# lukedan/libfluid

Hardware: AMD Instinct MI355X
Metric: particle_steps_per_sec (higher is better)
Workload: dtype f32

## Files before the change

### include/libfluid_amd.h

```cpp
#ifndef LIBFLUID_AMD_H
#define LIBFLUID_AMD_H

#include <stddef.h>
#include <stdint.h>

#ifdef __cplusplus
extern "C" {
#endif

typedef struct lfa_sim lfa_sim;

enum {
	LFA_OK = 0,
	LFA_E_INVALID = -1,
	LFA_E_NO_DEVICE = -2,
	LFA_E_HIP = -3,
	LFA_E_OOM = -4,
	LFA_E_NAN = -5,
	LFA_E_UNSUPPORTED = -6,
	LFA_W_PCG_NOT_CONVERGED = 1
};

enum { LFA_PIC = 0, LFA_FLIP_BLEND = 1, LFA_APIC = 2 };
enum { LFA_P2G_LDS_BINNED = 0, LFA_P2G_GLOBAL_ATOMIC = 1 };
// ... 80 lines not shown
int lfa_p2g(lfa_sim *s);
int lfa_add_gravity(lfa_sim *s, double dt);
int lfa_build_system(lfa_sim *s, double dt);
int lfa_download_abits(lfa_sim *s, uint8_t *bits, uint64_t n);
int lfa_download_rhs(lfa_sim *s, double *b, uint64_t n);
int lfa_download_precon(lfa_sim *s, double *precon, uint64_t n);
int lfa_apply_preconditioner(lfa_sim *s, const double *r, double *z, uint64_t n);
int lfa_apply_a(lfa_sim *s, const double *v, double *out, uint64_t n);
int lfa_pcg_solve(lfa_sim *s, double dt, double *residual, uint64_t *iterations);
int lfa_download_pressure(lfa_sim *s, double *p, uint64_t n);
int lfa_upload_pressure(lfa_sim *s, const double *p, uint64_t n);
int lfa_apply_pressure(lfa_sim *s, double dt);
int lfa_extrapolate(lfa_sim *s);
int lfa_g2p(lfa_sim *s);
int lfa_cfl(lfa_sim *s, double *out);

int lfa_step_hot(lfa_sim *s, double dt, double *residual, uint64_t *iterations);

int lfa_clear_sources(lfa_sim *s);
int lfa_add_source(lfa_sim *s, const int32_t *xyz, uint64_t k, const double velocity[3], uint64_t target_density_cubic_root,
                   int active, int coerce_velocity);
int lfa_update_sources(lfa_sim *s, uint64_t *n_seeded);
int lfa_update_sources_rng(lfa_sim *s, uint64_t *rng_state, int flags, uint64_t *n_seeded, double *positions,
                           uint64_t positions_capacity);
int lfa_set_source_rng(lfa_sim *s, int on, uint64_t rng_state, int flags);
int lfa_get_source_rng(const lfa_sim *s, int *on, uint64_t *rng_state);
int lfa_source_last(const lfa_sim *s, uint64_t out[3]);
int lfa_advect_collide(lfa_sim *s, double dt);
int lfa_correct_collide(lfa_sim *s, double dt);
int lfa_advect(lfa_sim *s, double dt);
int lfa_correct(lfa_sim *s, double dt);
int lfa_collide(lfa_sim *s);
int lfa_time_step(lfa_sim *s, double dt, double *residual, uint64_t *iterations);
#define LFA_NUM_STEP_TIMERS 16
int lfa_get_step_timings(lfa_sim *s, double ms[LFA_NUM_STEP_TIMERS]);
int lfa_set_step_overlap(lfa_sim *s, int on);
int lfa_correct_collide_begin(lfa_sim *s, double dt);
int lfa_correct_collide_end(lfa_sim *s);
int lfa_correct_collide_undo(lfa_sim *s);

int lfa_dist_unique_id(void *id128);
int lfa_dist_init_rccl(lfa_sim *s, int rank, int nranks, const void *id128, const int32_t *layer_bounds);
typedef struct lfa_hub lfa_hub;
lfa_hub *lfa_dist_local_hub_create(int nranks);
void lfa_dist_local_hub_destroy(lfa_hub *h);
int lfa_dist_init_local(lfa_sim *s, lfa_hub *h, int rank, const int32_t *layer_bounds);
int lfa_dist_init_shm(lfa_sim *s, const char *name, int rank, int nranks, const int32_t *layer_bounds);
int lfa_dist_get_slab(const lfa_sim *s, int32_t *lo, int32_t *hi);
int lfa_dist_abandon(lfa_sim *s);

typedef struct lfa_voxels lfa_voxels;
enum { LFA_VOX_INTERIOR = 0, LFA_VOX_EXTERIOR = 1, LFA_VOX_SURFACE = 2 };
int lfa_voxels_create(lfa_voxels **out, const uint64_t size[3], const double grid_offset[3], double cell_size, int device);
void lfa_voxels_destroy(lfa_voxels *v);
const char *lfa_voxels_last_error(const lfa_voxels *v);
int lfa_voxels_info(const lfa_voxels *v, int32_t grid_min[3], uint64_t size[3], double grid_offset[3], double *cell_size);
int lfa_voxels_upload(lfa_voxels *v, const uint8_t *types);
int lfa_voxels_download(lfa_voxels *v, uint8_t *types);
int lfa_voxels_voxelize_triangles(lfa_voxels *v, const double *positions, uint64_t n_vertices, const void *indices,
                                  int index_bytes, uint64_t n_indices);
int lfa_voxels_mark_exterior(lfa_voxels *v);
int lfa_voxelize_mesh(lfa_voxels **out, const double *positions, uint64_t n_vertices, const void *indices, int index_bytes,
                      uint64_t n_indices, double cell_size, const double ref_grid_offset[3], int device);
int lfa_voxels_count(lfa_voxels *v, int include_interior, int include_surface, const int64_t *ref_grid_size, uint64_t *count);
int lfa_voxels_cells(lfa_voxels *v, int include_interior, int include_surface, const int64_t *ref_grid_size, int32_t *xyz,
                     uint64_t capacity, uint64_t *count);
// ... 70 lines not shown
```

### libfluid_amd/__init__.py

```python
import ctypes as C
import os

import numpy as np

from . import scenes
from .scenes import CELL_DTYPE, PARTICLE_DTYPE

HERE = os.path.dirname(os.path.abspath(__file__))
LIB_PATH = os.path.join(HERE, "libfluid_amd.so")

PIC, FLIP_BLEND, APIC = 0, 1, 2
P2G_LDS_BINNED, P2G_GLOBAL_ATOMIC = 0, 1
PRECOND_MIC0_TILED, PRECOND_MIC0_EXACT, PRECOND_MULTILEVEL, PRECOND_MULTIGRID = 0, 1, 2, 3
PCG_F32, PCG_F64 = 0, 1
SEED_DRAW_LTR, SEED_COLLECTIVE = 1, 2
OK, W_PCG_NOT_CONVERGED = 0, 1
NUM_TIMERS = 10
NUM_STEP_TIMERS = 16
STEP_TIMER_NAMES = ["advect_collide", "bin", "p2g", "p2g_scatter_kernel", "build_system", "pcg_loop", "apply_pressure",
                    "correct_cell_index", "correct_tiled_kernel", "correct_collide", "extrapolate", "g2p", "time_step",
                    "pcg_iterations", "pcg_iteration_mean", "overlapped"]
TIMER_NAMES = ["bin", "p2g", "gravity", "build_system", "pcg_loop", "apply_pressure", "extrapolate", "g2p",
               "p2g_scatter_kernel", "pcg_iteration_mean"]

# ... 124 lines not shown
    "lfa_set_solid_from_voxels": (_int, [_vp, _vp, _int, _int]),
    "lfa_mesher_create": (_int, [C.POINTER(_vp), _vp, _vp, _dbl, _dbl, _u64, _int]),
    "lfa_mesher_create_window": (_int, [C.POINTER(_vp), _vp, _vp, _dbl, _dbl, _u64, _u64, _u64, _int]),
    "lfa_mesher_window": (_int, [_vp, C.POINTER(_u64), C.POINTER(_u64), C.POINTER(_u64), C.POINTER(_u64)]),
    "lfa_mesher_sample_ids": (_int, [_vp, _vp, _vp, _u64, _dbl]),
    "lfa_mesher_rebase": (_int, [_vp, _u64]),
    "lfa_mesher_destroy": (None, [_vp]),
    "lfa_mesher_last_error": (C.c_char_p, [_vp]),
    "lfa_mesher_sample": (_int, [_vp, _vp, _u64, _dbl]),
    "lfa_mesher_sample_sim": (_int, [_vp, _vp, _dbl]),
    "lfa_mesher_download_values": (_int, [_vp, _vp]),
    "lfa_mesher_upload_values": (_int, [_vp, _vp]),
    "lfa_mesher_marching_cubes": (_int, [_vp, C.POINTER(_u64), C.POINTER(_u64)]),
    "lfa_mesher_download_mesh": (_int, [_vp, _vp, _vp]),
    "lfa_mesher_normals": (_int, [_vp]),
    "lfa_mesher_download_normals": (_int, [_vp, _vp]),
    "lfa_mesher_normals_time": (_int, [_vp, C.POINTER(_dbl)]),
    "lfa_mesher_boundary_size": (_int, [_vp, C.POINTER(_u64), C.POINTER(_u64)]),
    "lfa_mesher_download_boundary": (_int, [_vp, _vp, _vp]),
    "lfa_mesher_window_normals": (_int, [_vp, _vp, _vp, _u64]),
    "lfa_mesher_window_normals_from": (_int, [_vp, _vp]),
    "lfa_mesher_vertex_velocities": (_int, [_vp, _vp, C.POINTER(_u64)]),
    "lfa_mesher_vertex_velocities_collective": (_int, [_vp, _vp, C.POINTER(_u64 * 2)]),
    "lfa_mesher_download_velocities": (_int, [_vp, _vp]),
    "lfa_mesher_velocities_time": (_int, [_vp, C.POINTER(_dbl)]),
    "lfa_clear_sources": (_int, [_vp]),
    "lfa_add_source": (_int, [_vp, _vp, _u64, _vp, _u64, _int, _int]),
    "lfa_update_sources": (_int, [_vp, C.POINTER(_u64)]),
    "lfa_update_sources_rng": (_int, [_vp, C.POINTER(_u64), _int, C.POINTER(_u64), _vp, _u64]),
    "lfa_set_source_rng": (_int, [_vp, _int, _u64, _int]),
    "lfa_get_source_rng": (_int, [_vp, C.POINTER(_int), C.POINTER(_u64)]),
    "lfa_source_last": (_int, [_vp, C.POINTER(_u64 * 3)]),
    "lfa_advect_collide": (_int, [_vp, _dbl]),
    "lfa_advect": (_int, [_vp, _dbl]),
    "lfa_correct": (_int, [_vp, _dbl]),
    "lfa_collide": (_int, [_vp]),
    "lfa_correct_collide": (_int, [_vp, _dbl]),
    "lfa_time_step": (_int, [_vp, _dbl, C.POINTER(_dbl), C.POINTER(_u64)]),
    "lfa_get_step_timings": (_int, [_vp, C.POINTER(_dbl * NUM_STEP_TIMERS)]),
    "lfa_set_step_overlap": (_int, [_vp, _int]),
    "lfa_get_correction_stats": (_int, [_vp, C.POINTER(_u64 * 2)]),
    "lfa_get_correction_stats_ex": (_int, [_vp, C.POINTER(_u64 * 3)]),
    "lfa_correct_collide_begin": (_int, [_vp, _dbl]),
    "lfa_correct_collide_end": (_int, [_vp]),
    "lfa_correct_collide_undo": (_int, [_vp]),
    "lfa_dist_unique_id": (_int, [_vp]),
    "lfa_dist_init_rccl": (_int, [_vp, _int, _int, _vp, _vp]),
    "lfa_dist_local_hub_create": (_vp, [_int]),
    "lfa_dist_local_hub_destroy": (None, [_vp]),
    "lfa_dist_init_local": (_int, [_vp, _vp, _int, _vp]),
    "lfa_dist_init_shm": (_int, [_vp, C.c_char_p, _int, _int, _vp]),
    "lfa_dist_get_slab": (_int, [_vp, C.POINTER(C.c_int32), C.POINTER(C.c_int32)]),
    "lfa_dist_abandon": (_int, [_vp]),
}
KERNELS = {"spmv_dot": 0, "axpy_max": 1, "mic_apply_dot": 2, "update_s": 3, "p2g_scatter": 4, "p2g_finalize": 5,
           "g2p": 6, "bin": 7, "mic_fine": 8, "coarse_levels": 9, "pcg_a": 10, "pcg_b": 11,
           "mg_axpy_presmooth": 12, "mg_down0": 13, "mg_coarse": 14, "mg_up0": 15}


def load_library():
    global _lib
    if _lib is None:
        path = os.environ.get("LFA_LIB_PATH") or LIB_PATH
        if not os.path.exists(path):
            raise ImportError(
                f"{path} is missing: build it with `python -c 'import __graft_entry__ as g; g.build()'` "
# ... 623 lines not shown
        cap, buf = 0, None
        if positions:
            cap = int(positions) if positions is not True else sum(getattr(self, "_source_targets", []))
            buf = np.empty((cap, 3), dtype=np.float64)
        self._chk(self.lib.lfa_update_sources_rng(self.h, C.byref(state), int(flags), C.byref(n),
                                                  None if buf is None else _ptr(buf), cap))
        return n.value, state.value, None if buf is None else buf[:n.value].copy()

    def set_source_rng(self, on, rng_state=0, flags=0):
        self._chk(self.lib.lfa_set_source_rng(self.h, int(bool(on)), int(rng_state), int(flags)))

    def source_last(self):
        out = (C.c_uint64 * 3)()
        self._chk(self.lib.lfa_source_last(self.h, C.byref(out)))
        return tuple(out)

    def get_source_rng(self):
        on, state = C.c_int(0), C.c_uint64(0)
        self._chk(self.lib.lfa_get_source_rng(self.h, C.byref(on), C.byref(state)))
        return bool(on.value), state.value

    def advect(self, dt):
        self._chk(self.lib.lfa_advect(self.h, float(dt)))

    def correct(self, dt):
        self._chk(self.lib.lfa_correct(self.h, float(dt)))

    def collide(self):
        self._chk(self.lib.lfa_collide(self.h))

    def advect_collide(self, dt):
        self._chk(self.lib.lfa_advect_collide(self.h, float(dt)))

    def correct_collide(self, dt):
        self._chk(self.lib.lfa_correct_collide(self.h, float(dt)))

    def correct_collide_begin(self, dt):
        self._chk(self.lib.lfa_correct_collide_begin(self.h, float(dt)))

    def correct_collide_end(self):
        self._chk(self.lib.lfa_correct_collide_end(self.h))

    def correct_collide_undo(self):
        self._chk(self.lib.lfa_correct_collide_undo(self.h))

    def time_step(self, dt):
        res, it = C.c_double(0.0), C.c_uint64(0)
        rc = self._chk(self.lib.lfa_time_step(self.h, float(dt), C.byref(res), C.byref(it)))
        return res.value, it.value, rc

    def step_timings(self):
        arr = (C.c_double * NUM_STEP_TIMERS)()
        self._chk(self.lib.lfa_get_step_timings(self.h, C.byref(arr)))
        return dict(zip(STEP_TIMER_NAMES, list(arr)))

    def correction_stats(self):
        arr = (C.c_uint64 * 2)()
        self._chk(self.lib.lfa_get_correction_stats(self.h, C.byref(arr)))
        return int(arr[0]), int(arr[1])

    def correction_stats_ex(self):
        arr = (C.c_uint64 * 3)()
        self._chk(self.lib.lfa_get_correction_stats_ex(self.h, C.byref(arr)))
        return int(arr[0]), int(arr[1]), int(arr[2])

    def set_step_overlap(self, on):
# ... 61 lines not shown
```

### libfluid_amd/csrc/common.h

```cpp
#pragma once

#include <hip/hip_runtime.h>
#include <stdint.h>

#include <string>
#include <vector>

#include "../../include/libfluid_amd.h"

hipError_t lfa_pool_malloc(void **p, size_t bytes);
hipError_t lfa_pool_free(void *p);
void lfa_pool_nosync_begin();
void lfa_pool_nosync_end();
template <typename T> inline hipError_t lfa_hip_malloc(T **p, size_t bytes) { return lfa_pool_malloc((void **)p, bytes); }
#define hipMalloc(p, n) lfa_hip_malloc((p), (n))
#define hipFree(p) lfa_pool_free((void *)(p))
struct lfa_stream_set;
lfa_stream_set *lfa_pool_take_set(int device);
void lfa_pool_park_set(lfa_stream_set *q);

#define LFA_TILE 8
#define LFA_TILE_CELLS 512
#define LFA_HALO 10
#define LFA_HALO_CELLS 1000
// ... 15 lines not shown
	uint32_t *id = nullptr;
	void *base = nullptr;
};

#define LFA_CLOSED_MAX_UNKNOWNS 64

struct GridDims {
	int nx, ny, nz;
	int ntx, nty, ntz;
	int nt;
};

struct lfa_knobs {
	int mg_no_persist = 0;
	int mg_dist_single = 0;
	int mg_co_fault = 0;
	int mg_no_top = 0;
	int mg_no_prune = 0;
	int mg_dist_levels = 0;
	int mg_no_closed = 0;
	int mg_no_tagged = 0;
};

struct lfa_sim {
	int device = 0;
	lfa_knobs knobs;
	hipStream_t stream = nullptr;
	hipStream_t stream2 = nullptr;
	hipEvent_t ev_fork = nullptr, ev_join = nullptr;
	hipStream_t stream3 = nullptr;
	hipEvent_t ev_cfork = nullptr, ev_cjoin = nullptr;
	bool overlap_correction = true;
	bool corr_in_flight = false;
	bool counts_fresh = false;
	bool move_pending = false;
	bool corr_begun = false;
	bool corr_undo_valid = false;
	uint32_t *corr_ovf = nullptr;
	int corr_parts_tiles = 0;
	GridDims g{};
	size_t nc = 0, ncp = 0;
	lfa_params prm{};
	std::string err;

	size_t np = 0, pcap = 0;
	ParticleSoA pb[2];
	int cur = 0;
	uint32_t *rank = nullptr;
	bool binned = false;

	struct lfa_dist *dist = nullptr;
	int slab_lo = 0, slab_hi = 0;
	int slab_align = 0;
	int *ptiles_all = nullptr;
	int p_off = 0, n_ptiles_all = 0;
	int n_own_first = 0, n_own_last = 0;
	int n_ghost_lo = 0, n_ghost_hi = 0;
	int *halo_tiles = nullptr;
	int n_halo[4] = {0, 0, 0, 0};
	void *xbuf[4] = {nullptr, nullptr, nullptr, nullptr};
	size_t xcap[4] = {0, 0, 0, 0};
	double *dist_red = nullptr;
	size_t np_live = 0;
	bool holes = false;
	size_t arrivals_at = 0, n_arrivals = 0;
	size_t ghost_at[2] = {0, 0}, n_ghost_particles = 0;

// ... 216 lines not shown
	return ip;
}

__device__ inline void cell_and_fraction(double pos, double off, double h, int n, int &cell, float &t) {
	double gp = (pos - off) / h;
	double m = gp < 0.0 ? 0.0 : gp;
	int c = m >= (double)n ? n - 1 : (int)m;
	if (c > n - 1) c = n - 1;
	double td = gp - (double)c;
	float tf = (float)td;
	if (!(tf > 0.0f)) tf = 0.0f;
	if (td < 1.0 && tf >= 1.0f) tf = 0.99999994f;
	if (tf > 1.0f) tf = 1.0f;
	cell = c;
	t = tf;
}

__device__ inline void particle_world_position(const GridDims &g, const IngestParams &ip, uint32_t b, float t0, float t1, float t2,
                                               double (&x)[3]) {
	int c[3];
	cell_coords(g, b, c);
	const float t[3] = {t0, t1, t2};
#pragma unroll
	for (int k = 0; k < 3; ++k) x[k] = ip.off[k] + ((double)c[k] + (double)t[k]) * ip.h;
}

__device__ inline void particle_zero_c_set_id(const ParticleSoA &p, size_t d, uint32_t id) {
#pragma unroll
	for (int k = 0; k < 9; ++k) p.c[k][d] = 0.0f;
	p.id[d] = id;
}

#define TC_CHUNKS 8
template <int CH>
__device__ inline void lfa_wave_tile_ranks(const uint32_t (&tile)[CH], uint32_t *tile_count, uint32_t (&my_rank)[CH]) {
	const int lane = threadIdx.x & 63;
	const unsigned long long lt = (1ull << lane) - 1ull;
	unsigned long long todo[CH];
#pragma unroll
	for (int c = 0; c < CH; ++c) {
		todo[c] = __ballot(tile[c] != 0xFFFFFFFFu);
		my_rank[c] = 0;
	}
	for (;;) {
		uint32_t t = 0xFFFFFFFFu;
		bool found = false;
#pragma unroll
		for (int c = 0; c < CH; ++c)
			if (!found && todo[c]) {
				t = __shfl(tile[c], __ffsll((long long)todo[c]) - 1, 64);
				found = true;
			}
		if (!found) break;
		unsigned long long same[CH];
		uint32_t total = 0;
#pragma unroll
		for (int c = 0; c < CH; ++c) {
			same[c] = __ballot(tile[c] == t) & todo[c];
			total += (uint32_t)__popcll(same[c]);
		}
		uint32_t base = 0;
		if (lane == 0) base = atomicAdd(&tile_count[t], total);
		base = __shfl(base, 0, 64);
#pragma unroll
		for (int c = 0; c < CH; ++c) {
			if ((same[c] >> lane) & 1ull) my_rank[c] = base + (uint32_t)__popcll(same[c] & lt);
			base += (uint32_t)__popcll(same[c]);
			todo[c] &= ~same[c];
		}
	}
}

__device__ inline float madd01(float c, float v, float s) { return __builtin_fmaf(c, v, s); }
__device__ inline double madd01(double c, double v, double s) { return __builtin_fma(c, v, s); }
__device__ inline float fma_r(float a, float b, float c) { return __builtin_fmaf(a, b, c); }
__device__ inline double fma_r(double a, double b, double c) { return __builtin_fma(a, b, c); }
__device__ inline double strided_partial_sum(const double *p, int n) {
	double v[8];
#pragma unroll
	for (int k = 0; k < 8; ++k) {
		const int i = (int)threadIdx.x + 256 * k;
		v[k] = i < n ? p[i] : 0.0;
	}
	double a = v[0];
#pragma unroll
	for (int k = 1; k < 8; ++k) a += v[k];
	for (int i = (int)threadIdx.x + 2048; i < n; i += 256) a += p[i];
	return a;
}
__device__ inline double strided_partial_max(const double *p, int n, bool &nan) {
	double v[8];
#pragma unroll
	for (int k = 0; k < 8; ++k) {
		const int i = (int)threadIdx.x + 256 * k;
		v[k] = i < n ? p[i] : -INFINITY;
	}
	double a = -INFINITY;
#pragma unroll
	for (int k = 0; k < 8; ++k) {
		nan |= v[k] != v[k];
		a = v[k] > a ? v[k] : a;
	}
	for (int i = (int)threadIdx.x + 2048; i < n; i += 256) {
// ... 2 lines not shown
		a = x > a ? x : a;
	}
	return a;
}
template <typename T> __device__ inline T wave_sum(T v) {
#pragma unroll
	for (int o = 32; o > 0; o >>= 1) v += __shfl_xor(v, o, 64);
	return v;
}
template <typename T> __device__ inline T wave_max(T v) {
#pragma unroll
	for (int o = 32; o > 0; o >>= 1) {
		T other = __shfl_xor(v, o, 64);
		v = other > v ? other : v;
	}
	return v;
}

int lfa_exclusive_scan_u32(lfa_sim *s, const uint32_t *in, uint32_t *out, size_t n, uint32_t *total_dev);
enum {
	LFA_PIN_SOURCE_TOTAL = 96,
	LFA_PIN_SEED_ACCEPTED = 97,
	LFA_PIN_SEED_OWNED = 98,
	LFA_PIN_RESIDENT = 99,
	LFA_PIN_SOURCE_TOTAL_ALL = 104,
	LFA_PIN_SOURCE_KEPT = 105,
	LFA_PIN_SAMPLE_OWNED = 106,
	LFA_PIN_SAMPLE_OUTSIDE = 107,
	LFA_PIN_TRACER_COUNTS = 108,
};
int lfa_scan_total(lfa_sim *s, const uint32_t *in, uint32_t *out, size_t n, uint32_t *total_dev, int slot, size_t *total);

int lfa_particles_alloc(lfa_sim *s, size_t n);
int lfa_hash_particles_impl(lfa_sim *s, bool counts_done);
int lfa_particles_materialize(lfa_sim *s);
int lfa_c_home_restore(lfa_sim *s);
int lfa_c_home_ensure(lfa_sim *s, size_t n);
int lfa_ensure_io(lfa_sim *s, size_t bytes);
int lfa_slab_download_slots(lfa_sim *s, const uint32_t **slot);
int lfa_sample_velocity_launch(lfa_sim *s, hipStream_t stream, const double *xyz, size_t n, const uint32_t *tile_rule, int z_lo, int z_hi,
                               double *velocity, uint8_t *types, uint32_t *counts_dev);
int lfa_sample_refresh(lfa_sim *s, const char *who, size_t room_bytes, const uint32_t **tile_rule, void **room, int *z_lo, int *z_hi);
int lfa_pcg_alloc(lfa_sim *s);
int lfa_number_unknowns(lfa_sim *s);

__host__ __device__ inline int lfa_stage_index(int hx, int hy, int hz) {
	return (unsigned)(hx - 1) < 8u ? (hx - 1) + 8 * (hy + 10 * hz) : 800 + (hx ? 100 : 0) + hy + 10 * hz;
}
__host__ __device__ inline int lfa_stage_source(int o) {
	if (o < 800) return 1 + (o & 7) + 10 * (o >> 3);
	const int q = o - 800, pl = q >= 100 ? 1 : 0, r = q - 100 * pl;
	return 9 * pl + 10 * r;
}

struct lfa_dist {
	int rank = 0, nranks = 1;
	int device_share = 1;
	int exchange(lfa_sim *s, const void *send_lo, size_t n_send_lo, void *recv_lo, size_t n_recv_lo, const void *send_hi,
	             size_t n_send_hi, void *recv_hi, size_t n_recv_hi) {
		++calls;
		return exchange_impl(s, send_lo, n_send_lo, recv_lo, n_recv_lo, send_hi, n_send_hi, recv_hi, n_recv_hi);
	}
	int allreduce(lfa_sim *s, double *dev, int count, bool is_max) {
		++calls;
		return allreduce_impl(s, dev, count, is_max);
	}
	int allreduce_buf(lfa_sim *s, void *dev, size_t count, int dtype, bool is_max) {
// ... 46 lines not shown
```

### libfluid_amd/csrc/core.hip

```cpp
#include <math.h>

#include <algorithm>
#include <stdarg.h>
#include <stdio.h>
#include <string.h>

#include <mutex>

#include "common.h"
#include "pcg.h"
#include "stream_set.h"

static thread_local std::string g_create_error;

int lfa_fail(lfa_sim *s, int code, const char *fmt, ...) {
	char buf[512];
	va_list ap;
	va_start(ap, fmt);
	vsnprintf(buf, sizeof buf, fmt, ap);
	va_end(ap);
	if (s) s->err = buf;
	else g_create_error = buf;
	return code;
}
// ... 1016 lines not shown
	if (s->c_home) {
		const hipError_t e = hipStreamSynchronize(s->stream);
		if (e != hipSuccess) return fail(e, "hipStreamSynchronize");
		LFA_HIP(s, hipFree(s->c_home));
	}
	s->c_home = nh;
	s->c_home_cap = cap;
	return LFA_OK;
}
int lfa_c_home_restore(lfa_sim *s) {
	if (!s->c_home_valid) return LFA_OK;
	s->c_home_valid = false;
	const size_t n = s->binned ? s->np_live : s->np;
	if (!n) return LFA_OK;
	hipLaunchKernelGGL(k_c_from_home, dim3((unsigned)((n + 255) / 256)), dim3(256), 0, s->stream, n, s->pb[s->cur], (const float *)s->c_home,
	                   s->c_home_cap);
	LFA_LAUNCH_CHECK(s);
	return LFA_OK;
}

int lfa_particles_materialize(lfa_sim *s) {
	if (!s->vc_pending) return LFA_OK;
	LFA_TRY(lfa_corr_commit(s));
	s->vc_pending = false;
	LFA_HIP(s, hipSetDevice(s->device));
	const size_t n = s->np_live;
	if (!n) return LFA_OK;
	hipLaunchKernelGGL(k_gather_vc, dim3((unsigned)((n + 255) / 256)), dim3(256), 0, s->stream, n, s->pb[s->cur ^ 1], s->pb[s->cur],
	                   (const uint32_t *)s->vc_src, s->vc_with_c ? 1 : 0);
	LFA_LAUNCH_CHECK(s);
	return LFA_OK;
}

extern "C" int lfa_hash_particles(lfa_sim *s) { return lfa_hash_particles_impl(s, false); }
int lfa_hash_particles_impl(lfa_sim *s, bool counts_done) {
	if (!s) return LFA_E_INVALID;
	LFA_HIP(s, hipSetDevice(s->device));
	LFA_TRY(lfa_corr_commit(s));
	LFA_TRY(lfa_particles_materialize(s));
	const GridDims &g = s->g;
	const int nt = g.nt, L = g.ntx * g.nty;
	const size_t n = s->binned ? s->np_live : s->np;
	ParticleSoA &src = s->pb[s->cur], &dst = s->pb[s->cur ^ 1];
	const int own_lo = s->slab_lo * L, own_hi = s->slab_hi * L;
	const int all_lo = lfa_has_lo(s) ? own_lo - L : own_lo, all_hi = lfa_has_hi(s) ? own_hi + L : own_hi;

	if (!counts_done) {
		LFA_HIP(s, hipMemsetAsync(s->tile_count, 0, (size_t)(nt + 1) * 4, s->stream));
		if (n) {
			hipLaunchKernelGGL(k_tile_count, dim3((unsigned)((n + 256 * TC_CHUNKS - 1) / (256 * TC_CHUNKS))), dim3(256), 0, s->stream, src.key, n,
			                   s->tile_count, s->rank);
			LFA_LAUNCH_CHECK(s);
		}
	}
	LFA_TRY(lfa_exclusive_scan_u32(s, s->tile_count, s->tile_start, (size_t)nt + 1, nullptr));
	LFA_HIP(s, hipMemcpyAsync(s->h_pinned + 8, s->tile_start + nt, 4, hipMemcpyDeviceToHost, s->stream));

	hipLaunchKernelGGL(k_tile_flags, dim3((nt + 255) / 256), dim3(256), 0, s->stream, s->tile_count, s->tile_flag, nt);
	LFA_LAUNCH_CHECK(s);
	LFA_TRY(lfa_dist_exchange_tile_layers_u32(s, s->tile_flag));
	hipLaunchKernelGGL(k_fill_i32, dim3((nt + 255) / 256), dim3(256), 0, s->stream, s->tile_pslot, nt, -1);
	LFA_LAUNCH_CHECK(s);
	const bool one_sync = !s->dist;
	if (one_sync) {
		uint32_t *tot = (uint32_t *)s->pcg_state + 8;
		LFA_TRY(compact_tiles_async(s, s->tile_flag, 0, nt, s->ptiles_all, s->tile_pslot, tot));
		LFA_HIP(s, hipMemsetAsync(s->tile_flag, 0, (size_t)(nt + 1) * 4, s->stream));
		hipLaunchKernelGGL(k_dilate_slots, dim3((nt + 255) / 256), dim3(256), 0, s->stream, (const int *)s->tile_pslot, s->tile_flag, g);
		LFA_LAUNCH_CHECK(s);
		LFA_TRY(compact_tiles_async(s, s->tile_flag, 0, nt, s->dtiles, nullptr, tot + 1));
		LFA_HIP(s, hipMemcpyAsync(s->h_pinned + 9, tot, 8, hipMemcpyDeviceToHost, s->stream));
		LFA_HIP(s, hipStreamSynchronize(s->stream));
		s->n_ptiles_all = (int)s->h_pinned[9];
		s->n_dtiles = (int)s->h_pinned[10];
		s->p_off = 0;
		s->n_ptiles = s->n_ptiles_all;
		s->n_own_first = s->n_own_last = s->n_ghost_lo = s->n_ghost_hi = 0;
		s->ptiles = s->ptiles_all;
	} else {
		uint32_t *tot = (uint32_t *)s->pcg_state + 20;
// ... 19 lines not shown
		}
		LFA_HIP(s, hipMemcpyAsync(s->h_pinned + 20, tot, 40, hipMemcpyDeviceToHost, s->stream));
		LFA_HIP(s, hipStreamSynchronize(s->stream));
		const uint32_t *h = s->h_pinned + 20;
		s->n_ptiles_all = (int)h[0];
		int vals[4];
		for (int k = 0; k < 4; ++k) vals[k] = marks[k] >= all_hi ? s->n_ptiles_all : (int)h[1 + k];
		s->p_off = vals[0];
		s->n_ptiles = vals[3] - vals[0];
		s->n_own_first = vals[1] - vals[0];
		s->n_own_last = vals[3] - vals[2];
		s->n_ghost_lo = s->p_off;
		s->n_ghost_hi = s->n_ptiles_all - vals[3];
		s->ptiles = s->ptiles_all + s->p_off;
		s->n_dtiles = (int)h[5];
		for (int w = 0; w < 4; ++w) s->n_halo[w] = (int)h[6 + w];
	}
	s->np_live = s->h_pinned[8];
	if (s->dist) s->np = s->np_live;
	s->holes = false;
	s->n_arrivals = 0;
	s->move_pending = false;
	if (n) {
		const dim3 sgrid((unsigned)((n + 255) / 256));
		const bool home = s->prm.simulation_method != LFA_APIC;
		if (home && !s->c_home_valid) {
			LFA_TRY(lfa_c_home_ensure(s, s->dist ? std::max<size_t>(s->pcap, (size_t)s->next_global_id) : s->pcap));
			hipLaunchKernelGGL(k_c_to_home, sgrid, dim3(256), 0, s->stream, n, src, s->c_home, s->c_home_cap);
			LFA_LAUNCH_CHECK(s);
			s->c_home_valid = true;
		} else if (!home && s->c_home_valid) {
			LFA_TRY(lfa_c_home_restore(s));
		}
		hipLaunchKernelGGL(k_tile_scatter, sgrid, dim3(256), 0, s->stream, n, src, dst, s->rank, s->tile_start, s->tile_count,
		                   s->binned ? 0 : 1, s->vc_src);
		LFA_LAUNCH_CHECK(s);
		s->cur ^= 1;
		s->vc_pending = true;
		s->vc_extent = n;
		s->vc_with_c = !home;
	}
	if (s->n_dtiles) {
		int grid = s->n_dtiles < 8192 ? s->n_dtiles : 8192;
		hipLaunchKernelGGL(k_cell_count, dim3(grid), dim3(256), 0, s->stream, s->dtiles, s->n_dtiles,
		                   s->pb[s->cur].key, s->tile_start, s->cell_count);
		LFA_LAUNCH_CHECK(s);
	}
	s->binned = true;
	s->system_valid = false;
	s->unknown_count_valid = false;
	return LFA_OK;
}

int lfa_dist_build_halo_lists(lfa_sim *s, const uint32_t *flag, int *lists, int n[4]) {
	const int L = s->g.ntx * s->g.nty;
	const int lo[4] = {s->slab_lo * L, (s->slab_hi - 1) * L, (s->slab_lo - 1) * L, s->slab_hi * L};
	const bool on[4] = {lfa_has_lo(s), lfa_has_hi(s), lfa_has_lo(s), lfa_has_hi(s)};
	uint32_t *tot = (uint32_t *)s->pcg_state + 26;
	LFA_HIP(s, hipMemsetAsync(tot, 0, 16, s->stream));
	for (int w = 0; w < 4; ++w)
		if (on[w]) LFA_TRY(compact_tiles_async(s, flag, lo[w], lo[w] + L, lists + (size_t)w * L, nullptr, tot + w));
	LFA_HIP(s, hipMemcpyAsync(s->h_pinned + 26, tot, 16, hipMemcpyDeviceToHost, s->stream));
	LFA_HIP(s, hipStreamSynchronize(s->stream));
	for (int w = 0; w < 4; ++w) n[w] = (int)s->h_pinned[26 + w];
	return LFA_OK;
}

__global__ void k_raw_unknown_flags(GridDims g, size_t nc, const uint32_t *cell_count, const uint32_t *tile_flag,
                                    uint32_t *flag, int z0, int z1) {
// ... 254 lines not shown
```

### libfluid_amd/csrc/particles.hip

```cpp
#include <math.h>

#include <algorithm>
#include <utility>

#include "common.h"
#include "pcg.h"

namespace {

__device__ inline bool solid_or_outside(const GridDims &g, const uint8_t *solid, int x, int y, int z) {
	if (!in_grid(g, x, y, z)) return true;
	return solid[blocked_index(g, x, y, z)] != 0;
}

__device__ inline void collide(const GridDims &g, const uint8_t *solid, double from[3], double to[3], double skin) {
	for (int bounce = 0; bounce < 3; ++bounce) {
		bool hit = false;
		double diff[3], inv[3], t[3];
		int cur[3], last[3], adv[3];
#pragma unroll
		for (int d = 0; d < 3; ++d) {
			cur[d] = (int)floor(from[d]);
			last[d] = (int)floor(to[d]);
			diff[d] = to[d] - from[d];
// ... 93 lines not shown
struct MoveParams {
	double dt_over_h;
	double skin;
	double corr;
	double inv_re2;
	float *c_home;
	size_t c_home_stride;
	int collide;
};

__global__ void __launch_bounds__(256) k_tile_has_solid(const uint8_t *solid, int nt, uint8_t *tile_solid) {
	for (int t = blockIdx.x; t < nt; t += gridDim.x) {
		const uint8_t *c = solid + (size_t)t * LFA_TILE_CELLS;
		const int any = __syncthreads_or((c[threadIdx.x] | c[threadIdx.x + 256]) != 0);
		if (threadIdx.x == 0) tile_solid[t] = (uint8_t)(any ? 1 : 0);
	}
}
__global__ void k_tile_clear(GridDims g, const uint8_t *tile_solid, uint8_t *tile_clear) {
	const int t = blockIdx.x * blockDim.x + threadIdx.x;
	if (t >= g.nt) return;
	int tx, ty, tz;
	tile_coords(g, t, tx, ty, tz);
	int any = 0;
	for (int dz = -1; dz <= 1; ++dz)
		for (int dy = -1; dy <= 1; ++dy)
			for (int dx = -1; dx <= 1; ++dx) {
				const int x = tx + dx, y = ty + dy, z = tz + dz;
				if ((unsigned)x < (unsigned)g.ntx && (unsigned)y < (unsigned)g.nty && (unsigned)z < (unsigned)g.ntz)
					any |= tile_solid[x + g.ntx * (y + g.nty * z)];
			}
	tile_clear[t] = (uint8_t)(any ? 0 : 1);
}

template <bool COERCE>
__device__ inline uint32_t advect_one(size_t i, const ParticleSoA &p, const GridDims &g, const uint8_t *solid, const MoveParams &mp,
                                      const uint8_t *coerce_map, const float *src_vel, const uint8_t *tile_clear) {
	const uint32_t key = p.key[i];
	if (key == 0xFFFFFFFFu) return key;
	int c[3];
	cell_of_key(g, key, c);
	const int nn[3] = {g.nx, g.ny, g.nz};
	float vel[3] = {p.v[0][i], p.v[1][i], p.v[2][i]};
	if (COERCE) {
		const uint32_t src = coerce_map[key];
		if (src) {
#pragma unroll
			for (int d = 0; d < 3; ++d) {
				vel[d] = src_vel[3 * (src - 1) + d];
				p.v[d][i] = vel[d];
			}
			if (mp.c_home) {
				const size_t j = p.id[i];
#pragma unroll
				for (int k = 0; k < 9; ++k) mp.c_home[k * mp.c_home_stride + j] = 0.0f;
			} else {
#pragma unroll
				for (int k = 0; k < 9; ++k) p.c[k][i] = 0.0f;
			}
		}
	}
	double from[3], to[3];
#pragma unroll
	for (int d = 0; d < 3; ++d) {
		from[d] = (double)c[d] + (double)p.t[d][i];
		double x = from[d] + (double)vel[d] * mp.dt_over_h;
		const double lo = mp.skin, hi = (double)nn[d] - mp.skin;
		to[d] = x < lo ? lo : (hi < x ? hi : x);
	}
	const bool open_water = (tile_clear[key >> 9] & 1) && fabs(to[0] - from[0]) < 7.0 && fabs(to[1] - from[1]) < 7.0 &&
	                        fabs(to[2] - from[2]) < 7.0;
	if (!open_water && mp.collide) collide(g, solid, from, to, mp.skin);
	int nc[3];
	float nt[3];
#pragma unroll
	for (int d = 0; d < 3; ++d) split_position(to[d], nn[d], nc[d], nt[d]);
	const uint32_t new_key = blocked_index(g, nc[0], nc[1], nc[2]);
	p.key[i] = new_key;
#pragma unroll
	for (int d = 0; d < 3; ++d) p.t[d][i] = nt[d];
	return new_key;
}

template <bool COERCE>
__global__ void __launch_bounds__(256)
k_advect_collide(size_t n, ParticleSoA p, GridDims g, const uint8_t *solid, MoveParams mp, const uint8_t *coerce_map,
                 const float *src_vel, const uint8_t *tile_clear) {
	const size_t i = (size_t)blockIdx.x * blockDim.x + threadIdx.x;
	if (i < n) advect_one<COERCE>(i, p, g, solid, mp, coerce_map, src_vel, tile_clear);
}

#define AC_CHUNKS 8
template <bool COERCE>
__global__ void __launch_bounds__(256)
k_advect_collide_count(size_t n, ParticleSoA p, GridDims g, const uint8_t *solid, MoveParams mp, const uint8_t *coerce_map,
                       const float *src_vel, const uint8_t *tile_clear, uint32_t *tile_count, uint32_t *rank) {
	const int lane = threadIdx.x & 63;
	const size_t wave = ((size_t)blockIdx.x * blockDim.x + threadIdx.x) >> 6;
	const size_t i0 = wave * (64 * AC_CHUNKS) + lane;
	uint32_t tile[AC_CHUNKS], my_rank[AC_CHUNKS];
#pragma unroll
	for (int c = 0; c < AC_CHUNKS; ++c) {
		const size_t i = i0 + 64 * c;
		const uint32_t k = i < n ? advect_one<COERCE>(i, p, g, solid, mp, coerce_map, src_vel, tile_clear) : 0xFFFFFFFFu;
		tile[c] = k != 0xFFFFFFFFu ? k >> 9 : 0xFFFFFFFFu;
	}
	lfa_wave_tile_ranks(tile, tile_count, my_rank);
#pragma unroll
	for (int c = 0; c < AC_CHUNKS; ++c) {
		const size_t i = i0 + 64 * c;
		if (tile[c] != 0xFFFFFFFFu) rank[i] = my_rank[c];
	}
}

__device__ inline float hash_unit(uint32_t a, uint32_t b, uint32_t k) {
	uint32_t x = a * 0x9E3779B1u ^ (b + 0x7F4A7C15u) * 0x85EBCA77u ^ k * 0xC2B2AE3Du;
	x ^= x >> 15; x *= 0x2C1B3C6Du; x ^= x >> 12; x *= 0x297A2D39u; x ^= x >> 15;
	return (float)(x >> 8) * (2.0f / 16777216.0f) - 1.0f;
}

#define FT 11
#define FTX (2 * FT)
#define FT3 (FTX * FT * FT)
#define FT_STRIDE (FT3 + 1)
#define FT_INV 1.375f
#define FTX_INV 2.75f
#define FT_PL ((FT + CORR_PARTS - 1) / CORR_PARTS)
#define FB 13
#define FBX (FTX + 4)
#define FBZ (FT_PL + 2)
#define FB_N (FBX * FB * FBZ)
#define FB_ROWS (FB * FBZ)
#define FINE_CAP 5632
#define FINE_CAP_BIG 12288
#define FIDX_THREADS 512
#define FIDX_CNT (((FT3 + 1 + FIDX_THREADS - 1) / FIDX_THREADS) * FIDX_THREADS)
#define FIDX_STAGE 4608

__device__ inline int fine_coord(int l, float t) {
	const int f = (int)(((float)l + t) * FT_INV);
	return f < FT - 1 ? f : FT - 1;
}
__device__ inline int fine_coord_x(int l, float t) {
	const int f = (int)(((float)l + t) * FTX_INV);
// ... 979 lines not shown
	if (on) *on = s->src_rng_on ? 1 : 0;
	if (rng_state) *rng_state = s->src_rng_state;
	return LFA_OK;
}

static int refresh_tile_clear(lfa_sim *s) {
	if (s->clear_epoch == s->solid_epoch && s->tile_clear) return LFA_OK;
	if (!s->tile_clear) LFA_HIP(s, hipMalloc(&s->tile_clear, (size_t)s->g.nt * 2));
	uint8_t *tile_solid = s->tile_clear + s->g.nt;
	hipLaunchKernelGGL(k_tile_has_solid, dim3(s->g.nt < 16384 ? s->g.nt : 16384), dim3(256), 0, s->stream, (const uint8_t *)s->solid,
	                   s->g.nt, tile_solid);
	hipLaunchKernelGGL(k_tile_clear, dim3((s->g.nt + 255) / 256), dim3(256), 0, s->stream, s->g, (const uint8_t *)tile_solid,
	                   s->tile_clear);
	LFA_LAUNCH_CHECK(s);
	s->clear_epoch = s->solid_epoch;
	return LFA_OK;
}

static int save_old_positions(lfa_sim *s, size_t n);
static int advect_collide(lfa_sim *s, double dt, bool with_count, bool split = false) {
	if (!s) return LFA_E_INVALID;
	LFA_HIP(s, hipSetDevice(s->device));
	LFA_TRY(lfa_corr_commit(s));
	LFA_TRY(lfa_particles_materialize(s));
	const size_t n = s->binned ? s->np_live : s->np;
	MoveParams mp = move_params(s, dt);
	s->move_pending = false;
	if (split) {
		LFA_TRY(save_old_positions(s, n));
		mp.collide = 0;
	}
	LFA_TRY(lfa_sources_sync(s));
	LFA_TRY(refresh_tile_clear(s));
	s->counts_fresh = false;
	if (n) {
		if (s->any_coerce) s->vmax2_valid = false;
		const uint8_t *cm = s->any_coerce ? (const uint8_t *)s->coerce_map : (const uint8_t *)nullptr;
		const float *sv = s->any_coerce ? (const float *)s->src_vel : (const float *)nullptr;
		if (with_count && !s->dist) {
			LFA_HIP(s, hipMemsetAsync(s->tile_count, 0, (size_t)(s->g.nt + 1) * 4, s->stream));
			const dim3 grid((unsigned)((n + 256 * AC_CHUNKS - 1) / (256 * AC_CHUNKS)));
			if (s->any_coerce)
				hipLaunchKernelGGL(k_advect_collide_count<true>, grid, dim3(256), 0, s->stream, n, s->pb[s->cur], s->g, s->solid,
				                   mp, cm, sv, (const uint8_t *)s->tile_clear, s->tile_count, s->rank);
			else
				hipLaunchKernelGGL(k_advect_collide_count<false>, grid, dim3(256), 0, s->stream, n, s->pb[s->cur], s->g, s->solid,
				                   mp, cm, sv, (const uint8_t *)s->tile_clear, s->tile_count, s->rank);
			s->counts_fresh = true;
		} else {
			const dim3 grid((unsigned)((n + 255) / 256));
			if (s->any_coerce)
				hipLaunchKernelGGL(k_advect_collide<true>, grid, dim3(256), 0, s->stream, n, s->pb[s->cur], s->g, s->solid, mp,
				                   cm, sv, (const uint8_t *)s->tile_clear);
			else
				hipLaunchKernelGGL(k_advect_collide<false>, grid, dim3(256), 0, s->stream, n, s->pb[s->cur], s->g, s->solid, mp,
				                   cm, sv, (const uint8_t *)s->tile_clear);
		}
		LFA_LAUNCH_CHECK(s);
	}
	if (!split) LFA_TRY(lfa_dist_migrate(s));
	s->unknown_count_valid = false;
	s->move_pending = split;
	return LFA_OK;
}
extern "C" int lfa_advect_collide(lfa_sim *s, double dt) { return advect_collide(s, dt, false); }
extern "C" int lfa_advect(lfa_sim *s, double dt) { return advect_collide(s, dt, false, true); }

namespace {
__global__ void __launch_bounds__(256)
k_collide_only(size_t n, ParticleSoA p, const uint32_t *old_key, const float *ot0, const float *ot1, const float *ot2, GridDims g,
               const uint8_t *solid, double skin) {
	const size_t i = (size_t)blockIdx.x * blockDim.x + threadIdx.x;
	if (i >= n) return;
	const uint32_t key = p.key[i];
	if (key == 0xFFFFFFFFu) return;
	const int nn[3] = {g.nx, g.ny, g.nz};
	int c[3], oc[3];
	cell_of_key(g, key, c);
	double from[3], to[3];
	const float ot[3] = {ot0 ? ot0[i] : p.t[0][i], ot1 ? ot1[i] : p.t[1][i], ot2 ? ot2[i] : p.t[2][i]};
	cell_of_key(g, old_key ? old_key[i] : key, oc);
#pragma unroll
	for (int d = 0; d < 3; ++d) {
		to[d] = (double)c[d] + (double)p.t[d][i];
		from[d] = (double)oc[d] + (double)ot[d];
	}
	collide(g, solid, from, to, skin);
	int nc[3];
	float nt[3];
#pragma unroll
	for (int d = 0; d < 3; ++d) split_position(to[d], nn[d], nc[d], nt[d]);
	p.key[i] = blocked_index(g, nc[0], nc[1], nc[2]);
#pragma unroll
	for (int d = 0; d < 3; ++d) p.t[d][i] = nt[d];
}
// ... 159 lines not shown
}

namespace {
__global__ void __launch_bounds__(256)
k_correct_undo(size_t n, const float4 *spos, const uint32_t *old_key, uint32_t *key, float *t0, float *t1, float *t2) {
	const size_t k = (size_t)blockIdx.x * blockDim.x + threadIdx.x;
	if (k >= n) return;
	const float4 rec = spos[k];
	const uint32_t i = __float_as_uint(rec.w);
	t0[i] = __uint_as_float(__float_as_uint(rec.x) & 0x3FFFFFFFu);
	t1[i] = __uint_as_float(__float_as_uint(rec.y) & 0x3FFFFFFFu);
	t2[i] = __uint_as_float(__float_as_uint(rec.z) & 0x3FFFFFFFu);
	key[k] = old_key[k];
}
}

extern "C" int lfa_correct_collide_undo(lfa_sim *s) {
	if (!s) return LFA_E_INVALID;
	if (!s->corr_begun) return LFA_OK;
	if (!s->corr_undo_valid)
		return lfa_fail(s, LFA_E_INVALID, "lfa_correct_collide_undo: positions, binning or solid cells have changed since lfa_correct_collide_begin");
	LFA_HIP(s, hipSetDevice(s->device));
	LFA_TRY(lfa_corr_commit(s));
	s->corr_begun = false;
	const size_t n = s->np_live;
	if (!n) return LFA_OK;
	ParticleSoA &cur = s->pb[s->cur], &oth = s->pb[s->cur ^ 1];
	hipLaunchKernelGGL(k_correct_undo, dim3((unsigned)((n + 255) / 256)), dim3(256), 0, s->stream, n, (const float4 *)correction_scratch(s),
	                   (const uint32_t *)oth.key, cur.key, cur.t[0], cur.t[1], cur.t[2]);
	LFA_LAUNCH_CHECK(s);
	return LFA_OK;
}

int lfa_g2p_stale(lfa_sim *s);
extern "C" int lfa_time_step(lfa_sim *s, double dt, double *residual, uint64_t *iterations) {
	if (!s) return LFA_E_INVALID;
	if (s->src_rng_on && s->dist && !(s->src_rng_flags & LFA_SEED_COLLECTIVE))
		return lfa_fail(s, LFA_E_UNSUPPORTED, "lfa_time_step: fluid sources that draw from the pcg32 (lfa_set_source_rng) on a slab decomposition");
	LFA_HIP(s, hipSetDevice(s->device));
	LFA_TRY(lfa_corr_commit(s));
	const bool tm = s->timing;
	enum { B_START = 24, B_ADVECT, B_BIN, B_P2G, B_SOLVE, B_APPLY, B_CORRECT, B_EXTRAP, B_G2P, B_JOIN };
	static_assert(B_CORRECT == LFA_EV_CORRECT_END, "event slot of the end of the correction");
	auto rec = [&](int id) -> int {
		if (tm) LFA_HIP(s, hipEventRecord(s->ev[id], s->stream));
		return LFA_OK;
	};
	LFA_TRY(rec(B_START));
	LFA_TRY(advect_collide(s, dt, true));
	LFA_TRY(rec(B_ADVECT));
	{
		const bool counted = s->counts_fresh;
		s->counts_fresh = false;
		LFA_TRY(lfa_hash_particles_impl(s, counted));
	}
	if (!s->sources.empty()) LFA_TRY(lfa_update_sources(s, nullptr));
	LFA_TRY(rec(B_BIN));
	const bool overlap = s->overlap_correction && (s->dist || s->np_live);
	LFA_TRY(lfa_p2g_run(s, true, dt));
	LFA_TRY(rec(B_P2G));
	if (overlap) {
		if (s->dist) LFA_TRY(lfa_dist_exchange_ghost_particles(s));
		LFA_TRY(correct_begin(s, dt, true));
	}
	double res = 0.0;
	uint64_t it = 0;
	int rc = LFA_OK;
	auto grid_stages = [&]() -> int {
		rc = lfa_pcg_solve(s, dt, &res, &it);
		if (rc < 0) return rc;
		LFA_TRY(rec(B_SOLVE));
		LFA_TRY(lfa_apply_pressure(s, dt));
		LFA_TRY(rec(B_APPLY));
		if (!overlap) {
			LFA_TRY(lfa_correct_collide(s, dt));
			LFA_TRY(rec(B_CORRECT));
		}
		LFA_TRY(lfa_extrapolate(s));
		return rec(B_EXTRAP);
	};
	const int rc_grid = grid_stages();
	if (overlap) LFA_TRY(lfa_corr_join(s));
	if (rc_grid < 0) return rc_grid;
	if (overlap && s->dist) LFA_TRY(lfa_dist_migrate(s, true));
	LFA_TRY(rec(B_JOIN));
	LFA_TRY(lfa_g2p_stale(s));
	if (tm) {
		LFA_TRY(rec(B_G2P));
// ... 83 lines not shown
```

Baseline: 5.283 billion.

## Defer particle advection into the binning scatter to avoid a write-then-reread pass

When the simulation is binned and single-device, advection now runs in a count-only kernel that computes new keys and adds to per-tile counts without writing positions back or recording ranks. The move is then recomputed inside a new scatter kernel that advects each particle again and writes it directly to its sorted slot, taking slots from per-tile cursors. This removes the in-place write of keys and positions plus the rank array traffic, at the cost of running the advection and collision math twice and using atomics for slot order, so particle order within a tile is no longer deterministic. A new lfa_step_advect_bin entry point exposes the fused path.

```diff
diff --git a/include/libfluid_amd.h b/include/libfluid_amd.h
--- a/include/libfluid_amd.h
+++ b/include/libfluid_amd.h
@@ -136,6 +136,7 @@
 int lfa_correct(lfa_sim *s, double dt);
 int lfa_collide(lfa_sim *s);
 int lfa_time_step(lfa_sim *s, double dt, double *residual, uint64_t *iterations);
+int lfa_step_advect_bin(lfa_sim *s, double dt);
 #define LFA_NUM_STEP_TIMERS 16
 int lfa_get_step_timings(lfa_sim *s, double ms[LFA_NUM_STEP_TIMERS]);
 int lfa_set_step_overlap(lfa_sim *s, int on);
diff --git a/libfluid_amd/__init__.py b/libfluid_amd/__init__.py
--- a/libfluid_amd/__init__.py
+++ b/libfluid_amd/__init__.py
@@ -180,6 +180,7 @@
     "lfa_get_source_rng": (_int, [_vp, C.POINTER(_int), C.POINTER(_u64)]),
     "lfa_source_last": (_int, [_vp, C.POINTER(_u64 * 3)]),
     "lfa_advect_collide": (_int, [_vp, _dbl]),
+    "lfa_step_advect_bin": (_int, [_vp, _dbl]),
     "lfa_advect": (_int, [_vp, _dbl]),
     "lfa_correct": (_int, [_vp, _dbl]),
     "lfa_collide": (_int, [_vp]),
@@ -869,6 +870,9 @@
     def advect_collide(self, dt):
         self._chk(self.lib.lfa_advect_collide(self.h, float(dt)))
 
+    def step_advect_bin(self, dt):
+        self._chk(self.lib.lfa_step_advect_bin(self.h, float(dt)))
+
     def correct_collide(self, dt):
         self._chk(self.lib.lfa_correct_collide(self.h, float(dt)))
 
diff --git a/libfluid_amd/csrc/common.h b/libfluid_amd/csrc/common.h
--- a/libfluid_amd/csrc/common.h
+++ b/libfluid_amd/csrc/common.h
@@ -71,7 +71,8 @@
 	hipEvent_t ev_cfork = nullptr, ev_cjoin = nullptr;
 	bool overlap_correction = true;
 	bool corr_in_flight = false;
-	bool counts_fresh = false;
+	int bin_pass1 = 0;
+	double owed_dt = 0.0;
 	bool move_pending = false;
 	bool corr_begun = false;
 	bool corr_undo_valid = false;
@@ -354,15 +355,15 @@
 }
 
 #define TC_CHUNKS 8
-template <int CH>
-__device__ inline void lfa_wave_tile_ranks(const uint32_t (&tile)[CH], uint32_t *tile_count, uint32_t (&my_rank)[CH]) {
+template <int CH, bool RANKS>
+__device__ inline void lfa_wave_tile_groups(const uint32_t (&tile)[CH], uint32_t *tile_count, uint32_t (&my_rank)[CH]) {
 	const int lane = threadIdx.x & 63;
 	const unsigned long long lt = (1ull << lane) - 1ull;
 	unsigned long long todo[CH];
 #pragma unroll
 	for (int c = 0; c < CH; ++c) {
 		todo[c] = __ballot(tile[c] != 0xFFFFFFFFu);
-		my_rank[c] = 0;
+		if (RANKS) my_rank[c] = 0;
 	}
 	for (;;) {
 		uint32_t t = 0xFFFFFFFFu;
@@ -382,15 +383,30 @@
 			total += (uint32_t)__popcll(same[c]);
 		}
 		uint32_t base = 0;
-		if (lane == 0) base = atomicAdd(&tile_count[t], total);
-		base = __shfl(base, 0, 64);
+		if (RANKS) {
+			if (lane == 0) base = atomicAdd(&tile_count[t], total);
+			base = __shfl(base, 0, 64);
+		} else if (lane == 0) {
+			atomicAdd(&tile_count[t], total);
+		}
 #pragma unroll
 		for (int c = 0; c < CH; ++c) {
-			if ((same[c] >> lane) & 1ull) my_rank[c] = base + (uint32_t)__popcll(same[c] & lt);
-			base += (uint32_t)__popcll(same[c]);
+			if (RANKS) {
+				if ((same[c] >> lane) & 1ull) my_rank[c] = base + (uint32_t)__popcll(same[c] & lt);
+				base += (uint32_t)__popcll(same[c]);
+			}
 			todo[c] &= ~same[c];
 		}
 	}
+}
+template <int CH>
+__device__ inline void lfa_wave_tile_ranks(const uint32_t (&tile)[CH], uint32_t *tile_count, uint32_t (&my_rank)[CH]) {
+	lfa_wave_tile_groups<CH, true>(tile, tile_count, my_rank);
+}
+template <int CH>
+__device__ inline void lfa_wave_tile_counts(const uint32_t (&tile)[CH], uint32_t *tile_count) {
+	uint32_t none[CH];
+	lfa_wave_tile_groups<CH, false>(tile, tile_count, none);
 }
 
 __device__ inline float madd01(float c, float v, float s) { return __builtin_fmaf(c, v, s); }
@@ -459,7 +475,9 @@
 int lfa_scan_total(lfa_sim *s, const uint32_t *in, uint32_t *out, size_t n, uint32_t *total_dev, int slot, size_t *total);
 
 int lfa_particles_alloc(lfa_sim *s, size_t n);
-int lfa_hash_particles_impl(lfa_sim *s, bool counts_done);
+enum { LFA_BIN_FULL = 0, LFA_BIN_COUNTED = 1, LFA_BIN_MOVE_OWED = 2 };
+int lfa_hash_particles_impl(lfa_sim *s, int pass1);
+int lfa_advect_scatter(lfa_sim *s, size_t n, const ParticleSoA &src, const ParticleSoA &dst);
 int lfa_particles_materialize(lfa_sim *s);
 int lfa_c_home_restore(lfa_sim *s);
 int lfa_c_home_ensure(lfa_sim *s, size_t n);
diff --git a/libfluid_amd/csrc/core.hip b/libfluid_amd/csrc/core.hip
--- a/libfluid_amd/csrc/core.hip
+++ b/libfluid_amd/csrc/core.hip
@@ -1072,8 +1072,8 @@
 	return LFA_OK;
 }
 
-extern "C" int lfa_hash_particles(lfa_sim *s) { return lfa_hash_particles_impl(s, false); }
-int lfa_hash_particles_impl(lfa_sim *s, bool counts_done) {
+extern "C" int lfa_hash_particles(lfa_sim *s) { return lfa_hash_particles_impl(s, LFA_BIN_FULL); }
+int lfa_hash_particles_impl(lfa_sim *s, int pass1) {
 	if (!s) return LFA_E_INVALID;
 	LFA_HIP(s, hipSetDevice(s->device));
 	LFA_TRY(lfa_corr_commit(s));
@@ -1085,7 +1085,7 @@
 	const int own_lo = s->slab_lo * L, own_hi = s->slab_hi * L;
 	const int all_lo = lfa_has_lo(s) ? own_lo - L : own_lo, all_hi = lfa_has_hi(s) ? own_hi + L : own_hi;
 
-	if (!counts_done) {
+	if (pass1 == LFA_BIN_FULL) {
 		LFA_HIP(s, hipMemsetAsync(s->tile_count, 0, (size_t)(nt + 1) * 4, s->stream));
 		if (n) {
 			hipLaunchKernelGGL(k_tile_count, dim3((unsigned)((n + 256 * TC_CHUNKS - 1) / (256 * TC_CHUNKS))), dim3(256), 0, s->stream, src.key, n,
@@ -1171,9 +1171,13 @@
 		} else if (!home && s->c_home_valid) {
 			LFA_TRY(lfa_c_home_restore(s));
 		}
-		hipLaunchKernelGGL(k_tile_scatter, sgrid, dim3(256), 0, s->stream, n, src, dst, s->rank, s->tile_start, s->tile_count,
-		                   s->binned ? 0 : 1, s->vc_src);
-		LFA_LAUNCH_CHECK(s);
+		if (pass1 == LFA_BIN_MOVE_OWED) {
+			LFA_TRY(lfa_advect_scatter(s, n, src, dst));
+		} else {
+			hipLaunchKernelGGL(k_tile_scatter, sgrid, dim3(256), 0, s->stream, n, src, dst, s->rank, s->tile_start, s->tile_count,
+			                   s->binned ? 0 : 1, s->vc_src);
+			LFA_LAUNCH_CHECK(s);
+		}
 		s->cur ^= 1;
 		s->vc_pending = true;
 		s->vc_extent = n;
diff --git a/libfluid_amd/csrc/particles.hip b/libfluid_amd/csrc/particles.hip
--- a/libfluid_amd/csrc/particles.hip
+++ b/libfluid_amd/csrc/particles.hip
@@ -149,14 +149,32 @@
 	tile_clear[t] = (uint8_t)(any ? 0 : 1);
 }
 
-template <bool COERCE>
-__device__ inline uint32_t advect_one(size_t i, const ParticleSoA &p, const GridDims &g, const uint8_t *solid, const MoveParams &mp,
-                                      const uint8_t *coerce_map, const float *src_vel, const uint8_t *tile_clear) {
-	const uint32_t key = p.key[i];
-	if (key == 0xFFFFFFFFu) return key;
+__device__ inline uint32_t advect_from(uint32_t key, const float (&t)[3], const float (&vel)[3], const GridDims &g, const uint8_t *solid,
+                                       const MoveParams &mp, const uint8_t *tile_clear, float (&nt)[3]) {
 	int c[3];
 	cell_of_key(g, key, c);
 	const int nn[3] = {g.nx, g.ny, g.nz};
+	double from[3], to[3];
+#pragma unroll
+	for (int d = 0; d < 3; ++d) {
+		from[d] = (double)c[d] + (double)t[d];
+		double x = from[d] + (double)vel[d] * mp.dt_over_h;
+		const double lo = mp.skin, hi = (double)nn[d] - mp.skin;
+		to[d] = x < lo ? lo : (hi < x ? hi : x);
+	}
+	const bool open_water = (tile_clear[key >> 9] & 1) && fabs(to[0] - from[0]) < 7.0 && fabs(to[1] - from[1]) < 7.0 &&
+	                        fabs(to[2] - from[2]) < 7.0;
+	if (!open_water && mp.collide) collide(g, solid, from, to, mp.skin);
+	int nc[3];
+#pragma unroll
+	for (int d = 0; d < 3; ++d) split_position(to[d], nn[d], nc[d], nt[d]);
+	return blocked_index(g, nc[0], nc[1], nc[2]);
+}
+template <bool COERCE>
+__device__ inline uint32_t advect_move(size_t i, const ParticleSoA &p, const GridDims &g, const uint8_t *solid, const MoveParams &mp,
+                                       const uint8_t *coerce_map, const float *src_vel, const uint8_t *tile_clear, float (&nt)[3]) {
+	const uint32_t key = p.key[i];
+	if (key == 0xFFFFFFFFu) return key;
 	float vel[3] = {p.v[0][i], p.v[1][i], p.v[2][i]};
 	if (COERCE) {
 		const uint32_t src = coerce_map[key];
@@ -176,22 +194,15 @@
 			}
 		}
 	}
-	double from[3], to[3];
-#pragma unroll
-	for (int d = 0; d < 3; ++d) {
-		from[d] = (double)c[d] + (double)p.t[d][i];
-		double x = from[d] + (double)vel[d] * mp.dt_over_h;
-		const double lo = mp.skin, hi = (double)nn[d] - mp.skin;
-		to[d] = x < lo ? lo : (hi < x ? hi : x);
-	}
-	const bool open_water = (tile_clear[key >> 9] & 1) && fabs(to[0] - from[0]) < 7.0 && fabs(to[1] - from[1]) < 7.0 &&
-	                        fabs(to[2] - from[2]) < 7.0;
-	if (!open_water && mp.collide) collide(g, solid, from, to, mp.skin);
-	int nc[3];
+	const float t[3] = {p.t[0][i], p.t[1][i], p.t[2][i]};
+	return advect_from(key, t, vel, g, solid, mp, tile_clear, nt);
+}
+template <bool COERCE>
+__device__ inline uint32_t advect_one(size_t i, const ParticleSoA &p, const GridDims &g, const uint8_t *solid, const MoveParams &mp,
+                                      const uint8_t *coerce_map, const float *src_vel, const uint8_t *tile_clear) {
 	float nt[3];
-#pragma unroll
-	for (int d = 0; d < 3; ++d) split_position(to[d], nn[d], nc[d], nt[d]);
-	const uint32_t new_key = blocked_index(g, nc[0], nc[1], nc[2]);
+	const uint32_t new_key = advect_move<COERCE>(i, p, g, solid, mp, coerce_map, src_vel, tile_clear, nt);
+	if (new_key == 0xFFFFFFFFu) return new_key;
 	p.key[i] = new_key;
 #pragma unroll
 	for (int d = 0; d < 3; ++d) p.t[d][i] = nt[d];
@@ -226,6 +237,71 @@
 	for (int c = 0; c < AC_CHUNKS; ++c) {
 		const size_t i = i0 + 64 * c;
 		if (tile[c] != 0xFFFFFFFFu) rank[i] = my_rank[c];
+	}
+}
+
+template <bool COERCE>
+__global__ void __launch_bounds__(256)
+k_advect_count(size_t n, ParticleSoA p, GridDims g, const uint8_t *solid, MoveParams mp, const uint8_t *coerce_map,
+               const float *src_vel, const uint8_t *tile_clear, uint32_t *tile_count) {
+	const int lane = threadIdx.x & 63;
+	const size_t wave = ((size_t)blockIdx.x * blockDim.x + threadIdx.x) >> 6;
+	const size_t i0 = wave * (64 * AC_CHUNKS) + lane;
+	uint32_t tile[AC_CHUNKS];
+#pragma unroll
+	for (int c = 0; c < AC_CHUNKS; ++c) {
+		const size_t i = i0 + 64 * c;
+		float nt[3];
+		const uint32_t k = i < n ? advect_move<COERCE>(i, p, g, solid, mp, coerce_map, src_vel, tile_clear, nt) : 0xFFFFFFFFu;
+		tile[c] = k != 0xFFFFFFFFu ? k >> 9 : 0xFFFFFFFFu;
+	}
+	lfa_wave_tile_counts(tile, tile_count);
+}
+
+#define SC_CHUNKS 4
+__global__ void __launch_bounds__(256)
+k_advect_scatter(size_t n, ParticleSoA src, ParticleSoA dst, GridDims g, const uint8_t *solid, MoveParams mp, const uint8_t *tile_clear,
+                 uint32_t *cursor, uint32_t *from) {
+	const int lane = threadIdx.x & 63;
+	const size_t wave = ((size_t)blockIdx.x * blockDim.x + threadIdx.x) >> 6;
+	const size_t i0 = wave * (64 * SC_CHUNKS) + lane;
+	uint32_t tile[SC_CHUNKS], key[SC_CHUNKS], id[SC_CHUNKS], slot[SC_CHUNKS];
+	float t[SC_CHUNKS][3], vel[SC_CHUNKS][3];
+#pragma unroll
+	for (int c = 0; c < SC_CHUNKS; ++c) {
+		const size_t i = i0 + 64 * c;
+		key[c] = 0xFFFFFFFFu;
+		if (i < n) {
+			key[c] = src.key[i];
+			id[c] = src.id[i];
+#pragma unroll
+			for (int k = 0; k < 3; ++k) {
+				t[c][k] = src.t[k][i];
+				vel[c][k] = src.v[k][i];
+			}
+		}
+	}
+#pragma unroll
+	for (int c = 0; c < SC_CHUNKS; ++c) {
+		tile[c] = 0xFFFFFFFFu;
+		if (key[c] != 0xFFFFFFFFu) {
+			float nt[3];
+			key[c] = advect_from(key[c], t[c], vel[c], g, solid, mp, tile_clear, nt);
+#pragma unroll
+			for (int k = 0; k < 3; ++k) t[c][k] = nt[k];
+			tile[c] = key[c] >> 9;
+		}
+	}
+	lfa_wave_tile_ranks(tile, cursor, slot);
+#pragma unroll
+	for (int c = 0; c < SC_CHUNKS; ++c) {
+		if (tile[c] == 0xFFFFFFFFu) continue;
+		const size_t d = slot[c];
+		dst.key[d] = key[c];
+#pragma unroll
+		for (int k = 0; k < 3; ++k) dst.t[k][d] = t[c][k];
+		dst.id[d] = id[c];
+		from[d] = (uint32_t)(i0 + 64 * c);
 	}
 }
 
@@ -1271,12 +1347,23 @@
 	}
 	LFA_TRY(lfa_sources_sync(s));
 	LFA_TRY(refresh_tile_clear(s));
-	s->counts_fresh = false;
+	s->bin_pass1 = LFA_BIN_FULL;
 	if (n) {
 		if (s->any_coerce) s->vmax2_valid = false;
 		const uint8_t *cm = s->any_coerce ? (const uint8_t *)s->coerce_map : (const uint8_t *)nullptr;
 		const float *sv = s->any_coerce ? (const float *)s->src_vel : (const float *)nullptr;
-		if (with_count && !s->dist) {
+		if (with_count && !s->dist && s->binned) {
+			LFA_HIP(s, hipMemsetAsync(s->tile_count, 0, (size_t)(s->g.nt + 1) * 4, s->stream));
+			const dim3 grid((unsigned)((n + 256 * AC_CHUNKS - 1) / (256 * AC_CHUNKS)));
+			if (s->any_coerce)
+				hipLaunchKernelGGL(k_advect_count<true>, grid, dim3(256), 0, s->stream, n, s->pb[s->cur], s->g, s->solid, mp, cm, sv,
+				                   (const uint8_t *)s->tile_clear, s->tile_count);
+			else
+				hipLaunchKernelGGL(k_advect_count<false>, grid, dim3(256), 0, s->stream, n, s->pb[s->cur], s->g, s->solid, mp, cm, sv,
+				                   (const uint8_t *)s->tile_clear, s->tile_count);
+			s->bin_pass1 = LFA_BIN_MOVE_OWED;
+			s->owed_dt = dt;
+		} else if (with_count && !s->dist) {
 			LFA_HIP(s, hipMemsetAsync(s->tile_count, 0, (size_t)(s->g.nt + 1) * 4, s->stream));
 			const dim3 grid((unsigned)((n + 256 * AC_CHUNKS - 1) / (256 * AC_CHUNKS)));
 			if (s->any_coerce)
@@ -1285,7 +1372,7 @@
 			else
 				hipLaunchKernelGGL(k_advect_collide_count<false>, grid, dim3(256), 0, s->stream, n, s->pb[s->cur], s->g, s->solid,
 				                   mp, cm, sv, (const uint8_t *)s->tile_clear, s->tile_count, s->rank);
-			s->counts_fresh = true;
+			s->bin_pass1 = LFA_BIN_COUNTED;
 		} else {
 			const dim3 grid((unsigned)((n + 255) / 256));
 			if (s->any_coerce)
@@ -1300,6 +1387,14 @@
 	if (!split) LFA_TRY(lfa_dist_migrate(s));
 	s->unknown_count_valid = false;
 	s->move_pending = split;
+	return LFA_OK;
+}
+int lfa_advect_scatter(lfa_sim *s, size_t n, const ParticleSoA &src, const ParticleSoA &dst) {
+	const MoveParams mp = move_params(s, s->owed_dt);
+	LFA_HIP(s, hipMemcpyAsync(s->tile_scan, s->tile_start, (size_t)s->g.nt * 4, hipMemcpyDeviceToDevice, s->stream));
+	hipLaunchKernelGGL(k_advect_scatter, dim3((unsigned)((n + 256 * SC_CHUNKS - 1) / (256 * SC_CHUNKS))), dim3(256), 0, s->stream, n, src, dst,
+	                   s->g, (const uint8_t *)s->solid, mp, (const uint8_t *)s->tile_clear, s->tile_scan, s->vc_src);
+	LFA_LAUNCH_CHECK(s);
 	return LFA_OK;
 }
 extern "C" int lfa_advect_collide(lfa_sim *s, double dt) { return advect_collide(s, dt, false); }
@@ -1525,6 +1620,17 @@
 	return LFA_OK;
 }
 
+static int bin_after_advect(lfa_sim *s) {
+	const int pass1 = s->bin_pass1;
+	s->bin_pass1 = LFA_BIN_FULL;
+	return lfa_hash_particles_impl(s, pass1);
+}
+extern "C" int lfa_step_advect_bin(lfa_sim *s, double dt) {
+	if (!s) return LFA_E_INVALID;
+	LFA_TRY(advect_collide(s, dt, true));
+	return bin_after_advect(s);
+}
+
 int lfa_g2p_stale(lfa_sim *s);
 extern "C" int lfa_time_step(lfa_sim *s, double dt, double *residual, uint64_t *iterations) {
 	if (!s) return LFA_E_INVALID;
@@ -1542,11 +1648,7 @@
 	LFA_TRY(rec(B_START));
 	LFA_TRY(advect_collide(s, dt, true));
 	LFA_TRY(rec(B_ADVECT));
-	{
-		const bool counted = s->counts_fresh;
-		s->counts_fresh = false;
-		LFA_TRY(lfa_hash_particles_impl(s, counted));
-	}
+	LFA_TRY(bin_after_advect(s));
 	if (!s->sources.empty()) LFA_TRY(lfa_update_sources(s, nullptr));
 	LFA_TRY(rec(B_BIN));
 	const bool overlap = s->overlap_correction && (s->dist || s->np_live);
```

New measurement: 5.323 billion (median of 6 runs). No clear change (+0.8%).
